# wreuven/h264-scroll-encoder

Measured on AMD Instinct MI355X. Metric: composed frames/sec (1280x720, 360x360 dyn) at 1/2/4/8 GPU; bit-exact vs CPU, higher is better.
Workload: dtype u8; 1 GPU; BASELINE config 3: 256 concurrent 1280x720 streams + 360x360 synthetic dynamic rect (4x4 int transform + quant + CAVLC), composer_write_scroll_frame semantics; resolution=1280x720, streams_per_gpu=256, parallelism=static stream shard x1, no RCCL

## Files before the change

h264-scroll-encoder_amd/csrc/dyn_engine.h:

```cpp
#ifndef SCROLL_DYN_ENGINE_H
#define SCROLL_DYN_ENGINE_H

#include <hip/hip_runtime.h>
#include "engine.h"

typedef struct {
    uint32_t *rows;
    uint16_t *meta;
    uint2 *body_lo, *body_hi;
    uint4 *body_w;
    uint4 *heads;
    unsigned long long *tcx;
    uint32_t *rowstage;
    uint32_t *gbits;
    uint32_t *spill;
    uint32_t *ctr;
    uint32_t ctr_frames;
    uint32_t epoch;
} DynScratch;
#define DYN_HEAD_VECS 16
#define DYN_CTR_LIST 4

typedef struct {
    hipStream_t side;
    hipEvent_t e0, e1;
} DynFork;
int dyn_launch_code(hipStream_t hs, int nframes, int S, DevStream *st, const NalDesc *nal,
                    int ld_nal, const PlanPending *pend, DynFrame *dfr, int ld_fr,
                    const DynGeom *g, const uint8_t *src, const uint8_t *refs, const DynScratch *x,
                    uint32_t epoch, int mbw, uint64_t *stamps, const DynFork *fk, hipEvent_t ev0 = nullptr,
                    hipEvent_t ev1 = nullptr);
int dyn_launch_static(hipStream_t hs, int nframes, int S, DevStream *st, const NalDesc *nal, int ld_nal,
                      const PlanPending *pend, DynFrame *dfr, int ld_fr, const DynGeom *g, const DynScratch *x);
int dyn_launch_pack(hipStream_t hs, int nframes, int S, DevStream *st, const NalDesc *nal,
                    int ld_nal, const PlanPending *pend, DynFrame *dfr, int ld_fr,
                    const DynGeom *g, const DynScratch *x, uint8_t *eps, uint64_t *stamps, const DynFork *fk);
int dyn_launch_emit(hipStream_t hs, int nframes, int S, const DevStream *st, const NalDesc *nal,
                    int ld_nal, const DynFrame *dfr, int ld_fr, const DynGeom *g,
                    const uint8_t *stage, const DynScratch *x, uint8_t *arena, uint64_t ld_arena,
                    uint64_t *stamps);
int dyn_launch_synth(hipStream_t hs, int nframes, int S, uint8_t *src, const DynGeom *g,
                     int stream_base, int t0);

void dyn_rowstage_geom(DynGeom *g, int mbw, int mbh);
size_t dyn_slot_bound(int mbw, int mbh, int rw, int rh);
uint32_t dyn_ep_cap(int rw, int rh, int debug);

#endif
```

h264-scroll-encoder_amd/csrc/dyn_kernels.hip:

```cpp
#include <hip/hip_runtime.h>

#include <stdint.h>
#include <mutex>

#include "dyn_device.h"
#include "dyn_engine.h"
#include "nal_ctx.h"
#include "row_mfma.h"
#include "stage_util.h"

using namespace scroll;
using namespace scroll::dyn;
using namespace scroll::stage;

namespace {

__constant__ Tabs g_tabs = SCROLL_DYN_TABS;
constexpr Tabs k_tabs = SCROLL_DYN_TABS;
__constant__ PTabs g_ptabs = make_ptabs(k_tabs);
__device__ uint32_t g_tzrb[TZRB_N];
__constant__ LvTab g_lvt = make_lvt();

struct QpPair {
    QParams l, c;
// ... 594 lines not shown

__device__ inline uint4 body_msb(uint64_t hi, uint64_t lo, uint32_t n)
{
    const uint32_t k = 128u - n;
    uint64_t H, Lw;
    if (k >= 64u) {
        H = k >= 128u ? 0ull : lo << (k - 64u);
        Lw = 0ull;
    } else {
        H = k ? (hi << k) | (lo >> (64u - k)) : hi;
        Lw = lo << k;
    }
    return make_uint4((uint32_t)(H >> 32), (uint32_t)H, (uint32_t)(Lw >> 32), (uint32_t)Lw);
}

__global__ __launch_bounds__(256) void k_dyn_rows(const DevStream *__restrict__ st,
                                                  const NalDesc *__restrict__ nal, int ld_nal,
                                                  const PlanPending *__restrict__ pend,
                                                  DynFrame *__restrict__ dfr, int ld_fr, DynGeom g,
                                                  uint32_t *__restrict__ rows, uint32_t *__restrict__ ctr,
                                                  uint4 *__restrict__ heads)
{
    __shared__ int32_t wo[8], wl[8], wv[8];
    __shared__ int32_t gen;
    const int s = blockIdx.y, f = blockIdx.x, t = threadIdx.x;
    DynFrame *DF = dfr + (size_t)s * ld_fr + f;
    const int j = DF->nal;
    if (j < 0) return;
    if (t < 8) {
        wo[t] = pend[s].wo[t];
        wl[t] = pend[s].wl[t];
        wv[t] = pend[s].wv[t];
    }
    if (t == 0) gen = 0;
    __syncthreads();
    const DevStream *S = st + s;
    const NalDesc d = nal[(size_t)s * ld_nal + j];
    const NalCtx c = nal_ctx(S, d, wo, wl, wv);
    if (t < 12) {
        const HeadCtx H = head_ctx(c);
        CapSink hc{0, 0, 0};
        H.put_class(hc, t);
        uint4 *hv = heads + ((size_t)s * ld_fr + f) * DYN_HEAD_VECS;
        hv[t] = body_msb(hc.hi, hc.lo, min(hc.n, 128u));
        reinterpret_cast<uint32_t *>(hv + 12)[t] = hc.n | (hc.over() ? 0x80000000u : 0u);
    }
    const Regions rg = regions(c);
    const int w = c.w, h = c.h, a_end = (h - c.off) / 16;
    const uint32_t ysz = (uint32_t)w * (uint32_t)h, pic = ysz + ysz / 2;
    const WpTab T{wo, wv, h};
    uint32_t *rw = rows + ((size_t)s * ld_fr + f) * (size_t)(32 * g.h);
    bool my_gen = false;
    for (int i = t; i < 32 * g.h; i += 256) {
        uint32_t e;
        if (i < 16 * g.h) {
            const int Y = 16 * g.y0 + i, row = Y >> 4;
            const bool cA = row < a_end;
            int yo;
            const int b = luma_row(T, cA ? rg.ra : rg.rb, Y + (cA ? rg.mva : rg.mvb), yo);
            e = (uint32_t)b * pic + (uint32_t)yo * (uint32_t)w;
        } else {
            const int i2 = i - 16 * g.h, bot = i2 >= 8 * g.h;
            const int Y = 8 * g.y0 + (bot ? i2 - 8 * g.h : i2), row = Y >> 3;
            const bool cA = row < a_end;
            const int q = 4 * (cA ? rg.mva : rg.mvb), o = q >> 3, fr = q & 7;
            int yo;
            const int b = chroma_row(T, cA ? rg.ra : rg.rb, Y + o + bot, yo);
            if (b < 0) {
// ... 10 lines not shown
    if (t == 0) {
        uint32_t e = 0u;
        if (gen) {
            const uint32_t k = atomicAdd(&ctr[1], 1u);
            if (k < g.gen_cap) {
                DF->rbsp_bytes = k;
                ctr[DYN_CTR_LIST + k] = (uint32_t)((size_t)s * ld_fr + f);
                e = DF_GENERAL;
            } else {
                e = DF_OVER;
            }
        }
        DF->err = e;
        DF->ep = 0u;
    }
}

constexpr int GW = 64;
#ifndef SCROLL_GBUF_WORDS
#define SCROLL_GBUF_WORDS 256
#endif
constexpr int GBUF_WORDS = SCROLL_GBUF_WORDS;

#ifndef SCROLL_STATIC_WORDS
#define SCROLL_STATIC_WORDS 1
#endif

struct StaticFixed {
    uint32_t ncand;
    uint32_t buf[GBUF_WORDS];
    uint64_t hhi[12], hlo[12];
    uint4 pat[12];
    uint32_t hlen[12];
    int32_t head_over;
    int32_t wo[8], wl[8], wv[8];
    uint32_t moff[DYN_STATIC_ROWS + 1];
};

__global__ __launch_bounds__(GW) void k_dyn_static(const DevStream *__restrict__ st,
                                                   const NalDesc *__restrict__ nal, int ld_nal,
                                                   const PlanPending *__restrict__ pend,
                                                   const DynFrame *__restrict__ dfr, int ld_fr, DynGeom g,
                                                   uint32_t *__restrict__ rowstage, uint32_t *__restrict__ gbits)
{
    __shared__ StaticFixed L;
    constexpr int SR = DYN_STATIC_ROWS;
    const Rect R{g.x0, g.y0, g.w, g.h};
    const int nA = max(1, (R.y0 + SR - 1) / SR);
    const int gi = (int)blockIdx.x >= nA ? (int)blockIdx.x + R.h : (int)blockIdx.x;
    const int ng = g.ngroups, f = blockIdx.y, s = blockIdx.z, t = threadIdx.x;
    const size_t nb = (size_t)s * ld_fr + f;
    const int j = dfr[nb].nal;
    if (j < 0) return;
    const bool first = gi == 0, last = gi == ng - 1;
    if (t < 8) {
        L.wo[t] = pend[s].wo[t];
        L.wl[t] = pend[s].wl[t];
        L.wv[t] = pend[s].wv[t];
    }
    if (t == 0) {
        L.head_over = 0;
        L.ncand = 0;
    }
    const DevStream *S = st + s;
    const NalDesc d = nal[(size_t)s * ld_nal + j];
    wave_sync();
    NalCtx c = nal_ctx(S, d, L.wo, L.wl, L.wv);
    c.qpd = S->dyn_qp - QP_DEFAULT;
    const HeadCtx H = head_ctx(c);
    const int mbw = H.mbw, mbh = c.h / 16;
    int ra, rb;
    if (gi < nA) {
        ra = gi * SR;
        rb = min(ra + SR, R.y0);
    } else {
        ra = R.y0 + R.h + (gi - nA - R.h) * SR;
        rb = min(ra + SR, mbh);
    }
    uint32_t F = 0;
    if (first) {
        CountSink hc{0};
        emit_slice_header(hc, c);
        F = hc.n;
    }
    if (t < 12) {
        CapSink hc{0, 0, 0};
        H.put_class(hc, t);
        L.hhi[t] = hc.hi;
        L.hlo[t] = hc.lo;
        L.hlen[t] = hc.n;
        if (hc.over()) L.head_over = 1;
        if (hc.n < 128u) {
            const uint64_t hi = (hc.hi << 1) | (hc.lo >> 63), lo = (hc.lo << 1) | 1u;
            L.pat[t] = body_msb(hi, lo, hc.n + 1u);
        } else {
            L.head_over = 1;
        }
    }
    wave_sync();
    const bool head_over = L.head_over;
    auto head_bits = [&](int r, int col) -> uint32_t {
        if (!head_over) return L.hlen[H.sel(r, col)];
        CountSink cn{0};
        H.put_slow(cn, r, col);
        return cn.n;
    };
    uint32_t len = 0;
    const int r = ra + t;
    if (r < rb) {
        if (!head_over) {
            len = row_static_bits(H, L.hlen, r, R);
        } else {
            for (int col = 0; col < mbw; ++col) len += head_bits(r, col) + 1u;
        }
    }
    const uint32_t incl = wave_incl_sum(len, t);
    if (r < rb) L.moff[r - ra] = F + incl - len;
    const uint32_t rows_end = F + __shfl(incl, GW - 1, GW);
    if (t == 0) L.moff[rb - ra] = rows_end;
    const uint32_t bits = rows_end + (last ? 1u : 0u);
    if (t == 0) gbits[nb * (size_t)ng + gi] = bits;
    wave_sync();

    uint32_t *out = rowstage + nb * g.rs_frame_words + rs_group_words(g, nA, gi);
    const uint32_t nw = min((bits + 31u) >> 5, g.rs_static_words - EPC_STATIC);
    const int ne = rb - ra;
    auto cnt_le = [&](uint32_t x) -> int {
        int lo = 0, hi = ne + 1;
        while (lo < hi) {
            const int mid = (lo + hi) >> 1;
            if (L.moff[mid] <= x) lo = mid + 1;
            else hi = mid;
        }
        return lo;
    };
    const uint32_t m_mbw = magic32((uint32_t)mbw);
    for (uint32_t p0 = 0; p0 < nw; p0 += GBUF_WORDS) {
        const uint32_t n = min((uint32_t)GBUF_WORDS, nw - p0);
        for (uint32_t i = (uint32_t)t; i < n; i += GW) L.buf[i] = 0u;
        wave_sync();
        const LdsOrWin win{L.buf, p0, n};
        if (!(SCROLL_STATIC_WORDS && !head_over) && first && t == 0 && p0 * 32u < F) {
            WSink hs{win, 0, 0, 0};
            hs.start(0);
            emit_slice_header(hs, c);
            hs.finish();
        }
        if (SCROLL_STATIC_WORDS && !head_over) {
            const uint32_t rbeg = L.moff[0], rend = L.moff[ne];
            for (uint32_t i = (uint32_t)t; i < n; i += GW) {
                const uint32_t W0 = 32u * (p0 + i), W1 = W0 + 32u;
                uint32_t acc = 0, b = max(W0, rbeg), R0 = 0, R1 = 0, L0 = 0, Lm = 1;
                int b3 = 0;
                float inv = 1.0f;
                while (b < W1 && b < rend) {
                    if (b >= R1 || b < R0) {
                        const int e = cnt_le(b) - 1;
                        R0 = L.moff[e];
                        R1 = L.moff[e + 1];
                        b3 = H.sel(ra + e, 0);
                        L0 = L.hlen[b3] + 1u;
                        Lm = L.hlen[b3 + 1] + 1u;
                        inv = 1.0f / (float)Lm;
                    }
                    const uint32_t o = b - R0;
                    uint32_t cl = (uint32_t)b3, off = o;
                    if (o >= L0) {
                        const uint32_t o2 = o - L0;
                        uint32_t q = (uint32_t)((float)o2 * inv);
                        if (q * Lm > o2) --q;
                        else if ((q + 1u) * Lm <= o2) ++q;
                        if (q < (uint32_t)(mbw - 2)) {
                            cl = (uint32_t)b3 + 1u;
                            off = o2 - q * Lm;
                        } else {
                            cl = (uint32_t)b3 + 2u;
                            off = o2 - (uint32_t)(mbw - 2) * Lm;
                        }
                    }
                    const uint32_t k = min(L.hlen[cl] + 1u - off, W1 - b);
                    const uint4 P = L.pat[cl];
                    const uint32_t wi = off >> 5, sh = off & 31u;
                    const uint32_t w0 = wi == 0 ? P.x : (wi == 1 ? P.y : (wi == 2 ? P.z : P.w));
                    const uint32_t w1 = wi == 0 ? P.y : (wi == 1 ? P.z : (wi == 2 ? P.w : 0u));
                    uint32_t v = sh ? __builtin_amdgcn_alignbit(w0, w1, 32u - sh) : w0;
                    v &= k >= 32u ? 0xffffffffu : ~(0xffffffffu >> k);
                    acc |= v >> (b - W0);
                    b += k;
                }
                L.buf[i] = acc;
            }
            wave_sync();
            if (first && t == 0 && p0 * 32u < F) {
                WSink hs{win, 0, 0, 0};
                hs.start(0);
                emit_slice_header(hs, c);
                hs.finish();
            }
            if (last && t == 0) {
                WSink sk{win, 0, 0, 0};
                sk.start(bits - 1u);
                sk.put(1, 1);
                sk.finish();
            }
            wave_sync();
            flush_window(L.buf, n, p0, p0 + n >= nw, out, &L.ncand,
                         rowstage + nb * g.rs_frame_words + rs_runs_words(g, nA, gi), EPC_STATIC - 1, t, GW);
            wave_sync();
            continue;
        }
        const int ea = max(cnt_le(32u * p0) - 1, 0), eb = min(cnt_le(32u * (p0 + n) - 1u), ne);
        const int nm = eb * mbw;
        for (int m = ea * mbw + t; m < nm; m += GW) {
            const int rr = (int)div_m((uint32_t)m, m_mbw), col = m - rr * mbw, rw = ra + rr;
            uint32_t off = L.moff[rr];
            WSink sk{win, 0, 0, 0};
            if (!head_over) {
                const int b3 = H.sel(rw, 0);
                off += col == 0 ? 0u : L.hlen[b3] + 1u + (uint32_t)(col - 1) * (L.hlen[b3 + 1] + 1u);
                if (off >= 32u * (p0 + n)) continue;
                const int cls = b3 + (col == 0 ? 0 : (col == mbw - 1 ? 2 : 1));
                if (off + L.hlen[cls] + 1u <= 32u * p0) continue;
                sk.start(off);
                sk.put_cap(CapSink{L.hhi[cls], L.hlo[cls], L.hlen[cls]});
            } else {
                for (int c2 = 0; c2 < col; ++c2) off += head_bits(rw, c2) + 1u;
                sk.start(off);
                H.put_slow(sk, rw, col);
            }
            sk.put(1, 1);
            sk.finish();
        }
        if (last && t == 0) {
            WSink sk{win, 0, 0, 0};
            sk.start(bits - 1u);
            sk.put(1, 1);
            sk.finish();
        }
        wave_sync();
        flush_window(L.buf, n, p0, p0 + n >= nw, out, &L.ncand,
                     rowstage + nb * g.rs_frame_words + rs_runs_words(g, nA, gi), EPC_STATIC - 1, t, GW);
        wave_sync();
    }
    if (t == 0) rowstage[nb * g.rs_frame_words + rs_runs_words(g, nA, gi)] = L.ncand;
}


__device__ inline CapSink cap_of_msb(uint64_t a, uint64_t b, uint32_t n)
{
    if (n == 0u) return CapSink{0, 0, 0};
    const uint32_t sh = 128u - n;
    if (sh >= 64u) return CapSink{0, a >> (sh - 64u), n};
    if (sh == 0u) return CapSink{a, b, n};
    return CapSink{a >> sh, (b >> sh) | (a << (64u - sh)), n};
}

__device__ inline void put_piece(uint32_t *buf, uint32_t p0, uint32_t n, uint32_t pos, uint32_t tv, uint32_t tl,
                                 uint4 b, uint32_t bl)
{
    const uint32_t tw = tv & low_mask((int)tl);
    const uint32_t c0 = __builtin_amdgcn_alignbit(tw, b.x, tl), c1 = __builtin_amdgcn_alignbit(b.x, b.y, tl);
// ... 2359 lines not shown
    } else {
        const uint32_t r = (i - ly) % (64u * (uint32_t)g.w * (uint32_t)g.h);
        const int cw = 8 * g.w;
        const int y = (int)(r / (uint32_t)cw), x = (int)(r - (uint32_t)(y * cw));
        const int X = 8 * g.x0 + x, Y = 8 * g.y0 + y;
        v = 128 + ((X + Y + (int)tt) & 15) - 8 + (int)(hv >> 30);
    }
    src[(size_t)s * g.src_ld + (size_t)f * g.src_fr + i] = (uint8_t)clampi(v, 0, 255);
}

}

int dyn_launch_code(hipStream_t hs, int nframes, int S, DevStream *st, const NalDesc *nal,
                    int ld_nal, const PlanPending *pend, DynFrame *dfr, int ld_fr,
                    const DynGeom *g, const uint8_t *src, const uint8_t *refs, const DynScratch *x,
                    uint32_t epoch, int mbw, uint64_t *stamps, const DynFork *fk, hipEvent_t ev0, hipEvent_t ev1)
{
    if (nframes <= 0 || S <= 0) return 0;
    {
        static std::mutex mu;
        static uint64_t ready = 0;
        int dev = 0;
        if (hipGetDevice(&dev) != hipSuccess || dev >= 64) return -1;
        std::lock_guard<std::mutex> lk(mu);
        if (!(ready >> dev & 1u)) {
            hipLaunchKernelGGL(k_tzrb_init, dim3((TZRB_N + 255) / 256), dim3(256), 0, hs);
            if (hipGetLastError() != hipSuccess || hipStreamSynchronize(hs) != hipSuccess) return -1;
            ready |= 1ull << dev;
        }
    }
    hipLaunchKernelGGL(k_dyn_rows, dim3(nframes, S), dim3(256), 0, hs, st, nal, ld_nal, pend, dfr, ld_fr,
                       *g, x->rows, x->ctr, x->heads);
    if (hipGetLastError() != hipSuccess) return -1;
    hipStream_t hg = hs;
    if (fk) {
        if (hipEventRecord(fk->e0, hs) != hipSuccess || hipStreamWaitEvent(fk->side, fk->e0, 0) != hipSuccess)
            return -1;
        hg = fk->side;
    }
    const int nchunk = (24 * g->w * g->h + CODE_T - 1) / CODE_T;
    hipLaunchKernelGGL(k_dyn_code_general, dim3(nchunk, CODE_GEN_Y), dim3(CODE_T), 0, hg, st, dfr, ld_fr,
                       pend, nal, ld_nal, *g, x->rows, src, refs, x->meta, x->body_lo, x->body_hi, x->body_w,
                       x->ctr);
    if (hipGetLastError() != hipSuccess) return -1;
    if (row_lds_bytes(g->w) > 65536) {
        const int rl = (int)row_lds_bytes(g->w);
        if (hipFuncSetAttribute(reinterpret_cast<const void *>(&k_dyn_row<false>),
                                hipFuncAttributeMaxDynamicSharedMemorySize, rl) != hipSuccess ||
            hipFuncSetAttribute(reinterpret_cast<const void *>(&k_dyn_row<true>),
                                hipFuncAttributeMaxDynamicSharedMemorySize, rl) != hipSuccess)
            return -1;
    }
    if (ev0 && hipEventRecord(ev0, hs) != hipSuccess) return -1;
    hipLaunchKernelGGL(k_dyn_row<false>, dim3(g->h, nframes, S), dim3(row_threads(g->w)),
                       row_lds_bytes(g->w), hs, st, nal, ld_nal, pend, dfr, ld_fr, *g, x->rows, src, refs,
                       x->meta, x->body_lo, x->body_hi, x->body_w, x->tcx, epoch, x->rowstage, x->gbits, x->spill,
                       x->ctr, x->heads, stamps);
    if (hipGetLastError() != hipSuccess) return -1;
    if (ev1 && hipEventRecord(ev1, hs) != hipSuccess) return -1;
    hipLaunchKernelGGL(k_dyn_row<true>, dim3(g->h, std::min<uint32_t>(g->gen_cap, (uint32_t)(nframes * S)), 1),
                       dim3(row_threads(g->w)),
                       row_lds_bytes(g->w), hg, st, nal, ld_nal, pend, dfr, ld_fr, *g, x->rows, src, refs,
                       x->meta, x->body_lo, x->body_hi, x->body_w, x->tcx, epoch, x->rowstage, x->gbits, x->spill,
                       x->ctr, x->heads, stamps);
    if (hipGetLastError() != hipSuccess) return -1;
    if (fk) {
        if (dyn_launch_static(hg, nframes, S, st, nal, ld_nal, pend, dfr, ld_fr, g, x) ||
            hipEventRecord(fk->e1, hg) != hipSuccess)
            return -1;
    }
    return 0;
}

int dyn_launch_static(hipStream_t hs, int nframes, int S, DevStream *st, const NalDesc *nal, int ld_nal,
                      const PlanPending *pend, DynFrame *dfr, int ld_fr, const DynGeom *g, const DynScratch *x)
{
    if (nframes <= 0 || S <= 0) return 0;
    hipLaunchKernelGGL(k_dyn_static, dim3(g->ngroups - g->h, nframes, S), dim3(GW), 0, hs, st, nal, ld_nal,
                       pend, dfr, ld_fr, *g, x->rowstage, x->gbits);
    return hipGetLastError() == hipSuccess ? 0 : -1;
}

int dyn_launch_pack(hipStream_t hs, int nframes, int S, DevStream *st, const NalDesc *nal,
                    int ld_nal, const PlanPending *pend, DynFrame *dfr, int ld_fr,
                    const DynGeom *g, const DynScratch *x, uint8_t *eps, uint64_t *stamps, const DynFork *fk)
{
    if (nframes <= 0 || S <= 0) return 0;
    if (fk) {
        if (hipStreamWaitEvent(hs, fk->e1, 0) != hipSuccess) return -1;
    } else if (dyn_launch_static(hs, nframes, S, st, nal, ld_nal, pend, dfr, ld_fr, g, x)) {
        return -1;
    }
    if (g->ep_cap >= (uint32_t)EPF_BIG_LIST)
        hipLaunchKernelGGL((k_dyn_epfix<EPF_T, EPF_BIG_LIST>), dim3(nframes, S), dim3(EPF_T), gtab_bytes(g->ngroups, true),
                           hs, st, dfr, ld_fr, nframes, *g, x->rowstage, x->gbits, eps, stamps);
    else
        hipLaunchKernelGGL((k_dyn_epfix<EPF_T, EPF_LIST>), dim3(nframes, S), dim3(EPF_T), gtab_bytes(g->ngroups, true),
                           hs, st, dfr, ld_fr, nframes, *g, x->rowstage, x->gbits, eps, stamps);
    return hipGetLastError() == hipSuccess ? 0 : -1;
}

int dyn_launch_emit(hipStream_t hs, int nframes, int S, const DevStream *st, const NalDesc *nal,
                    int ld_nal, const DynFrame *dfr, int ld_fr, const DynGeom *g,
                    const uint8_t *stage, const DynScratch *x, uint8_t *arena, uint64_t ld_arena,
                    uint64_t *stamps)
{
    if (nframes <= 0 || S <= 0) return 0;
// ... 70 lines not shown
```

h264-scroll-encoder_amd/csrc/scroll_kernels.hip:

```cpp
#include <hip/hip_runtime.h>

#include <stdarg.h>
#include <stdint.h>
#include <stdio.h>
#include <stdlib.h>
#include <string.h>

#include <algorithm>
#include <mutex>
#include <vector>

#include "dyn_engine.h"
#include "recon_engine.h"
#include "hrecon_engine.h"
#include "hint_engine.h"
#include "splice_engine.h"
#include "hdyn_engine.h"
#include "ingest_engine.h"
#include "ipcm_engine.h"
#include "engine.h"
#include "scroll_device.h"

#include "dyn_device.h"

// ... 809 lines not shown
    int hint_max_mb = 0;
    std::vector<std::vector<ScrollHintRect>> h_hint;
    std::vector<int16_t> h_hint_mode;
    HintFrame *d_hf = nullptr;
    ScrollHintRect *d_pool = nullptr;
    size_t pool_cap = 0;
    struct SpliceHost {
        int x0 = 0, y0 = 0, w = 0, h = 0;
        std::vector<uint8_t> nal;
        const uint8_t *dnal = nullptr;
        size_t n = 0;
    };
    std::vector<SpliceHost> h_sp;
    std::vector<int32_t> h_dyn_pos;
    int fallback = 0;
    DynFork fork{};
    std::vector<int32_t> h_dyn_qp;
    int dyn_pos_custom = 0;
    int dyn_qp = 26;
    int hd_dirty = 0;
    uint32_t hd_mb_words = 0;
    size_t dyn_cap = 0;
    int sp_n = 0;
    int sp_dirty = 0;
    int sp_parse = 0;
    SpliceFrame *d_spf = nullptr;
    uint8_t *d_sp_nal = nullptr;
    uint32_t *d_sp_rbsp = nullptr;
    SpliceMbRec *d_sp_rec = nullptr;
    int32_t *d_sp_list = nullptr;
    SpliceUnit *d_sp_units = nullptr;
// ... 124 lines not shown
    }
    memset(b->h_st, 0, S * sizeof(DevStream));
    b->last = b->own;
    *out = b;
    return SCROLL_OK;
}

void scroll_batch_destroy(ScrollBatch *b)
{
    if (!b) return;
    (void)hipSetDevice(b->device);
    if (b->own) (void)hipStreamSynchronize(b->own);
    for (int i = 0; i < NEV; ++i)
        if (b->ev[i]) (void)hipEventDestroy(b->ev[i]);
    for (hipEvent_t e : b->ring) (void)hipEventDestroy(e);
    if (b->fork.side) {
        (void)hipStreamSynchronize(b->fork.side);
        (void)hipStreamDestroy(b->fork.side);
        (void)hipEventDestroy(b->fork.e0);
        (void)hipEventDestroy(b->fork.e1);
    }
    if (b->own) (void)hipStreamDestroy(b->own);
    (void)hipFree(b->d_st);
    (void)hipHostFree(b->h_st);
    (void)hipFree(b->d_off);
    (void)hipFree(b->d_nal);
    (void)hipFree(b->d_arena);
    (void)hipFree(b->d_out_tab);
    (void)hipFree(b->d_upd);
    if (b->out_ev) (void)hipEventDestroy(b->out_ev);
    (void)hipFree(b->d_pend);
    (void)hipFree(b->d_dfr);
    (void)hipFree(b->d_src);
    (void)hipFree(b->d_refs);
    (void)hipFree(b->d_stage);
    (void)hipFree(b->d_rec);
// ... 278 lines not shown
                b->rc_timed = timed ? 1 : 0;
                b->rc_last_hint = 1;
                std::fill(b->rc_fail.begin(), b->rc_fail.end(), 0);
            }
            if ((b->sp_n > 0 || combined) &&
                splice_launch_stage(hs, nframes, S, b->d_st, b->d_nal, b->ld_nal, b->d_pend,
                                    b->d_dfr, ld_fr, b->d_hf, b->d_pool, b->d_spf, b->d_sp_rec,
                                    b->d_sp_rbsp, b->d_stage, b->geo.slot_bytes)) {
                set_err("k_splice_stage launch: %s", hipGetErrorString(hipGetLastError()));
                return SCROLL_ERR_HIP;
            }
            if ((rc = mark(6))) return rc;
        } else {
            b->dx.epoch = b->dx.epoch % 0xffffffu + 1u;
            const DynGeom &G = b->geo;
            const DynFork *fk = nullptr;
            static const bool fork_on = [] {
                const char *e = getenv("SCROLL_DYN_FORK");
                return e && e[0] == '1';
            }();
            if (fork_on) {
                if (!b->fork.side) {
                    HIPCHK(hipStreamCreateWithFlags(&b->fork.side, hipStreamNonBlocking));
                    HIPCHK(hipEventCreateWithFlags(&b->fork.e0, hipEventDisableTiming));
                    HIPCHK(hipEventCreateWithFlags(&b->fork.e1, hipEventDisableTiming));
                }
                fk = &b->fork;
            }
            if (dyn_launch_code(hs, nframes, S, b->d_st, b->d_nal, b->ld_nal, b->d_pend, b->d_dfr, ld_fr, &G,
                                b->d_src, b->d_refs, &b->dx, b->dx.epoch, b->dyn_pw / 16, stamps, fk,
                                lite_row ? rev[1] : nullptr, lite_row ? rev[6] : nullptr)) {
                set_err("k_dyn_code launch: %s", hipGetErrorString(hipGetLastError()));
                return SCROLL_ERR_HIP;
            }
            if ((rc = mark(6))) return rc;
            if (b->recon_on) {
                const bool timed = b->timing != 0;
                if (timed && !b->rc_ev[0]) {
                    HIPCHK(hipEventCreate(&b->rc_ev[0]));
                    HIPCHK(hipEventCreate(&b->rc_ev[1]));
                }
                if (recon_launch(hs, nframes, S, b->d_st, b->d_nal, b->ld_nal, b->d_pend, b->d_dfr, ld_fr, &G,
                                 b->dx.rows, b->d_src, b->d_refs, b->d_rec, b->d_sse, b->dx.ctr,
                                 timed ? b->rc_ev[0] : nullptr, timed ? b->rc_ev[1] : nullptr)) {
                    set_err("k_dyn_recon launch: %s", hipGetErrorString(hipGetLastError()));
                    return SCROLL_ERR_HIP;
                }
                b->rc_timed = timed ? 1 : 0;
                b->rc_last_hint = 0;
            }
            if (dyn_launch_pack(hs, nframes, S, b->d_st, b->d_nal, b->ld_nal, b->d_pend, b->d_dfr, ld_fr, &G,
                                &b->dx, b->d_stage, stamps ? b->d_dbg : nullptr, fk)) {
                set_err("k_dyn_static / k_dyn_epfix launch: %s", hipGetErrorString(hipGetLastError()));
                return SCROLL_ERR_HIP;
            }
        }
        if ((rc = mark(2))) return rc;
        hipLaunchKernelGGL(k_plan, dim3(S), dim3(PLAN_THREADS), 0, hs, b->d_st, b->d_off,
                           b->max_frames, b->d_nal, b->ld_nal, nframes, plan_mode,
                           b->debug | plan_flags | PLAN_SIZE | PLAN_DYN, b->d_pend, b->d_dfr,
                           ld_fr, (b->dyn_on && !b->hint_on) ? (const uint32_t *)b->dx.ctr : nullptr,
                           b->geo.rs_spill_cap, b->geo.gen_cap);
        HIPCHK(hipGetLastError());
        if ((rc = mark(3))) return rc;
    }
    int per_wg = EMIT_WAVES * TILE;
    int gx = (nal_max + per_wg - 1) / per_wg;
    if (gx > 0 && (b->debug & SCROLL_DEBUG_EMIT_STAMPS)) {
// ... 2161 lines not shown
```

Before: 2.875 million frames/s.

## Fuse static-group bitstream packing into k_dyn_rows and drop the side-stream fork

The separate k_dyn_static kernel, one 64-thread block per static row group, frame and stream, is folded into k_dyn_rows. The per-frame head classes are now computed once per block into shared StaticHeads, and each wave then processes static groups with its own dynamically sized LDS window. A precomputed repeated-pattern table (rep) lets the middle macroblocks of a row be copied in 32-bit chunks instead of pattern by pattern. The optional SCROLL_DYN_FORK side-stream path is removed. This cuts one launch and the repeated head-context setup per group, but the static work now runs serially before the general coder instead of possibly overlapping with it, and k_dyn_rows uses a variable block size chosen by rows_threads.

```diff
diff --git a/h264-scroll-encoder_amd/csrc/dyn_engine.h b/h264-scroll-encoder_amd/csrc/dyn_engine.h
--- a/h264-scroll-encoder_amd/csrc/dyn_engine.h
+++ b/h264-scroll-encoder_amd/csrc/dyn_engine.h
@@ -21,20 +21,13 @@
 #define DYN_HEAD_VECS 16
 #define DYN_CTR_LIST 4
 
-typedef struct {
-    hipStream_t side;
-    hipEvent_t e0, e1;
-} DynFork;
 int dyn_launch_code(hipStream_t hs, int nframes, int S, DevStream *st, const NalDesc *nal,
                     int ld_nal, const PlanPending *pend, DynFrame *dfr, int ld_fr,
                     const DynGeom *g, const uint8_t *src, const uint8_t *refs, const DynScratch *x,
-                    uint32_t epoch, int mbw, uint64_t *stamps, const DynFork *fk, hipEvent_t ev0 = nullptr,
+                    uint32_t epoch, int mbw, uint64_t *stamps, hipEvent_t ev0 = nullptr,
                     hipEvent_t ev1 = nullptr);
-int dyn_launch_static(hipStream_t hs, int nframes, int S, DevStream *st, const NalDesc *nal, int ld_nal,
-                      const PlanPending *pend, DynFrame *dfr, int ld_fr, const DynGeom *g, const DynScratch *x);
-int dyn_launch_pack(hipStream_t hs, int nframes, int S, DevStream *st, const NalDesc *nal,
-                    int ld_nal, const PlanPending *pend, DynFrame *dfr, int ld_fr,
-                    const DynGeom *g, const DynScratch *x, uint8_t *eps, uint64_t *stamps, const DynFork *fk);
+int dyn_launch_pack(hipStream_t hs, int nframes, int S, DevStream *st, DynFrame *dfr, int ld_fr,
+                    const DynGeom *g, const DynScratch *x, uint8_t *eps, uint64_t *stamps);
 int dyn_launch_emit(hipStream_t hs, int nframes, int S, const DevStream *st, const NalDesc *nal,
                     int ld_nal, const DynFrame *dfr, int ld_fr, const DynGeom *g,
                     const uint8_t *stage, const DynScratch *x, uint8_t *arena, uint64_t ld_arena,
diff --git a/h264-scroll-encoder_amd/csrc/dyn_kernels.hip b/h264-scroll-encoder_amd/csrc/dyn_kernels.hip
--- a/h264-scroll-encoder_amd/csrc/dyn_kernels.hip
+++ b/h264-scroll-encoder_amd/csrc/dyn_kernels.hip
@@ -632,15 +632,267 @@
     return make_uint4((uint32_t)(H >> 32), (uint32_t)H, (uint32_t)(Lw >> 32), (uint32_t)Lw);
 }
 
-__global__ __launch_bounds__(256) void k_dyn_rows(const DevStream *__restrict__ st,
+constexpr int GW = 64;
+#ifndef SCROLL_GBUF_WORDS
+#define SCROLL_GBUF_WORDS 256
+#endif
+constexpr int GBUF_WORDS = SCROLL_GBUF_WORDS;
+
+#ifndef SCROLL_STATIC_WORDS
+#define SCROLL_STATIC_WORDS 1
+#endif
+
+struct StaticHeads {
+    uint64_t hhi[12], hlo[12];
+    uint4 pat[12];
+    uint32_t hlen[12];
+    uint32_t rep[4][5];
+    int32_t head_over;
+};
+struct StaticWave {
+    uint32_t ncand;
+    uint32_t buf[GBUF_WORDS];
+    uint32_t moff[DYN_STATIC_ROWS + 1];
+};
+
+__device__ inline void static_rep_put(uint32_t *rp, uint4 P, uint32_t L)
+{
+    rp[0] = P.x;
+    rp[1] = P.y;
+    rp[2] = P.z;
+    rp[3] = P.w;
+    rp[4] = 0u;
+    for (uint32_t n = L; n < 160u; n <<= 1) {
+        const int ws = (int)(n >> 5);
+        const uint32_t bs = n & 31u;
+        uint32_t sft[5];
+#pragma unroll
+        for (int j = 0; j < 5; ++j) {
+            const int a = j - ws;
+            const uint32_t lo = a >= 0 ? rp[a] : 0u, hi = a >= 1 ? rp[a - 1] : 0u;
+            sft[j] = bs ? __builtin_amdgcn_alignbit(hi, lo, bs) : lo;
+        }
+#pragma unroll
+        for (int j = 0; j < 5; ++j) rp[j] |= sft[j];
+    }
+}
+
+__device__ inline void static_heads_put(StaticHeads &HD, int k, const CapSink &hc)
+{
+    HD.hhi[k] = hc.hi;
+    HD.hlo[k] = hc.lo;
+    HD.hlen[k] = hc.n;
+    if (hc.over()) HD.head_over = 1;
+    if (hc.n < 128u) {
+        const uint64_t hi = (hc.hi << 1) | (hc.lo >> 63), lo = (hc.lo << 1) | 1u;
+        HD.pat[k] = body_msb(hi, lo, hc.n + 1u);
+        if (k % 3 == 1) static_rep_put(HD.rep[k / 3], HD.pat[k], hc.n + 1u);
+    } else {
+        HD.head_over = 1;
+    }
+}
+
+__device__ inline void static_group(const StaticHeads &HD, StaticWave &L, const NalCtx &c, const HeadCtx &H,
+                                    const DynGeom &g, size_t nb, int gi, uint32_t *__restrict__ rowstage,
+                                    uint32_t *__restrict__ gbits, int t)
+{
+    constexpr int SR = DYN_STATIC_ROWS;
+    const Rect R{g.x0, g.y0, g.w, g.h};
+    const int nA = max(1, (R.y0 + SR - 1) / SR);
+    const int ng = g.ngroups;
+    const bool first = gi == 0, last = gi == ng - 1;
+    if (t == 0) L.ncand = 0;
+    const int mbw = H.mbw, mbh = c.h / 16;
+    int ra, rb;
+    if (gi < nA) {
+        ra = gi * SR;
+        rb = min(ra + SR, R.y0);
+    } else {
+        ra = R.y0 + R.h + (gi - nA - R.h) * SR;
+        rb = min(ra + SR, mbh);
+    }
+    uint32_t F = 0;
+    if (first) {
+        CountSink hc{0};
+        emit_slice_header(hc, c);
+        F = hc.n;
+    }
+    const bool head_over = HD.head_over;
+    auto head_bits = [&](int r, int col) -> uint32_t {
+        if (!head_over) return HD.hlen[H.sel(r, col)];
+        CountSink cn{0};
+        H.put_slow(cn, r, col);
+        return cn.n;
+    };
+    uint32_t len = 0;
+    const int r = ra + t;
+    if (r < rb) {
+        if (!head_over) {
+            len = row_static_bits(H, HD.hlen, r, R);
+        } else {
+            for (int col = 0; col < mbw; ++col) len += head_bits(r, col) + 1u;
+        }
+    }
+    const uint32_t incl = wave_incl_sum(len, t);
+    if (r < rb) L.moff[r - ra] = F + incl - len;
+    const uint32_t rows_end = F + __shfl(incl, GW - 1, GW);
+    if (t == 0) L.moff[rb - ra] = rows_end;
+    const uint32_t bits = rows_end + (last ? 1u : 0u);
+    if (t == 0) gbits[nb * (size_t)ng + gi] = bits;
+    wave_sync();
+
+    uint32_t *out = rowstage + nb * g.rs_frame_words + rs_group_words(g, nA, gi);
+    const uint32_t nw = min((bits + 31u) >> 5, g.rs_static_words - EPC_STATIC);
+    const int ne = rb - ra;
+    auto cnt_le = [&](uint32_t x) -> int {
+        int lo = 0, hi = ne + 1;
+        while (lo < hi) {
+            const int mid = (lo + hi) >> 1;
+            if (L.moff[mid] <= x) lo = mid + 1;
+            else hi = mid;
+        }
+        return lo;
+    };
+    const uint32_t m_mbw = magic32((uint32_t)mbw);
+    for (uint32_t p0 = 0; p0 < nw; p0 += GBUF_WORDS) {
+        const uint32_t n = min((uint32_t)GBUF_WORDS, nw - p0);
+        for (uint32_t i = (uint32_t)t; i < n; i += GW) L.buf[i] = 0u;
+        wave_sync();
+        const LdsOrWin win{L.buf, p0, n};
+        if (!(SCROLL_STATIC_WORDS && !head_over) && first && t == 0 && p0 * 32u < F) {
+            WSink hs{win, 0, 0, 0};
+            hs.start(0);
+            emit_slice_header(hs, c);
+            hs.finish();
+        }
+        if (SCROLL_STATIC_WORDS && !head_over) {
+            const uint32_t rbeg = L.moff[0], rend = L.moff[ne];
+            for (uint32_t i = (uint32_t)t; i < n; i += GW) {
+                const uint32_t W0 = 32u * (p0 + i), W1 = W0 + 32u;
+                uint32_t acc = 0, b = max(W0, rbeg), R0 = 0, R1 = 0, L0 = 0, Lm = 1;
+                int b3 = 0;
+                float inv = 1.0f;
+                while (b < W1 && b < rend) {
+                    if (b >= R1 || b < R0) {
+                        const int e = cnt_le(b) - 1;
+                        R0 = L.moff[e];
+                        R1 = L.moff[e + 1];
+                        b3 = H.sel(ra + e, 0);
+                        L0 = HD.hlen[b3] + 1u;
+                        Lm = HD.hlen[b3 + 1] + 1u;
+                        inv = 1.0f / (float)Lm;
+                    }
+                    const uint32_t o = b - R0;
+                    uint32_t cl = (uint32_t)b3, off = o;
+                    if (o >= L0) {
+                        const uint32_t o2 = o - L0, mid = (uint32_t)max(mbw - 2, 0) * Lm;
+                        if (o2 < mid) {
+                            uint32_t q = (uint32_t)((float)o2 * inv);
+                            if (q * Lm > o2) --q;
+                            else if ((q + 1u) * Lm <= o2) ++q;
+                            const uint32_t ph = o2 - q * Lm, k = min(mid - o2, W1 - b);
+                            const uint32_t *rp = HD.rep[b3 / 3];
+                            const uint32_t wi = ph >> 5, sh = ph & 31u;
+                            const uint32_t w0 = rp[wi], w1 = rp[wi + 1u];
+                            uint32_t v = sh ? __builtin_amdgcn_alignbit(w0, w1, 32u - sh) : w0;
+                            v &= k >= 32u ? 0xffffffffu : ~(0xffffffffu >> k);
+                            acc |= v >> (b - W0);
+                            b += k;
+                            continue;
+                        }
+                        cl = (uint32_t)b3 + 2u;
+                        off = o2 - mid;
+                    }
+                    const uint32_t k = min(HD.hlen[cl] + 1u - off, W1 - b);
+                    const uint4 P = HD.pat[cl];
+                    const uint32_t wi = off >> 5, sh = off & 31u;
+                    const uint32_t w0 = wi == 0 ? P.x : (wi == 1 ? P.y : (wi == 2 ? P.z : P.w));
+                    const uint32_t w1 = wi == 0 ? P.y : (wi == 1 ? P.z : (wi == 2 ? P.w : 0u));
+                    uint32_t v = sh ? __builtin_amdgcn_alignbit(w0, w1, 32u - sh) : w0;
+                    v &= k >= 32u ? 0xffffffffu : ~(0xffffffffu >> k);
+                    acc |= v >> (b - W0);
+                    b += k;
+                }
+                L.buf[i] = acc;
+            }
+            wave_sync();
+            if (first && t == 0 && p0 * 32u < F) {
+                WSink hs{win, 0, 0, 0};
+                hs.start(0);
+                emit_slice_header(hs, c);
+                hs.finish();
+            }
+            if (last && t == 0) {
+                WSink sk{win, 0, 0, 0};
+                sk.start(bits - 1u);
+                sk.put(1, 1);
+                sk.finish();
+            }
+            wave_sync();
+            flush_window(L.buf, n, p0, p0 + n >= nw, out, &L.ncand,
+                         rowstage + nb * g.rs_frame_words + rs_runs_words(g, nA, gi), EPC_STATIC - 1, t, GW);
+            wave_sync();
+            continue;
+        }
+        const int ea = max(cnt_le(32u * p0) - 1, 0), eb = min(cnt_le(32u * (p0 + n) - 1u), ne);
+        const int nm = eb * mbw;
+        for (int m = ea * mbw + t; m < nm; m += GW) {
+            const int rr = (int)div_m((uint32_t)m, m_mbw), col = m - rr * mbw, rw = ra + rr;
+            uint32_t off = L.moff[rr];
+            WSink sk{win, 0, 0, 0};
+            if (!head_over) {
+                const int b3 = H.sel(rw, 0);
+                off += col == 0 ? 0u : HD.hlen[b3] + 1u + (uint32_t)(col - 1) * (HD.hlen[b3 + 1] + 1u);
+                if (off >= 32u * (p0 + n)) continue;
+                const int cls = b3 + (col == 0 ? 0 : (col == mbw - 1 ? 2 : 1));
+                if (off + HD.hlen[cls] + 1u <= 32u * p0) continue;
+                sk.start(off);
+                sk.put_cap(CapSink{HD.hhi[cls], HD.hlo[cls], HD.hlen[cls]});
+            } else {
+                for (int c2 = 0; c2 < col; ++c2) off += head_bits(rw, c2) + 1u;
+                sk.start(off);
+                H.put_slow(sk, rw, col);
+            }
+            sk.put(1, 1);
+            sk.finish();
+        }
+        if (last && t == 0) {
+            WSink sk{win, 0, 0, 0};
+            sk.start(bits - 1u);
+            sk.put(1, 1);
+            sk.finish();
+        }
+        wave_sync();
+        flush_window(L.buf, n, p0, p0 + n >= nw, out, &L.ncand,
+                     rowstage + nb * g.rs_frame_words + rs_runs_words(g, nA, gi), EPC_STATIC - 1, t, GW);
+        wave_sync();
+    }
+    if (t == 0) rowstage[nb * g.rs_frame_words + rs_runs_words(g, nA, gi)] = L.ncand;
+    wave_sync();
+}
+
+constexpr int ROWS_MAXW = 8, ROWS_SLOTS = 8192;
+inline int rows_threads(const DynGeom &g, int64_t nnal)
+{
+    const int nst = g.ngroups - g.h;
+    int64_t maxw = nnal > 0 ? ROWS_SLOTS / nnal : ROWS_MAXW;
+    maxw = maxw < 1 ? 1 : (maxw > ROWS_MAXW ? ROWS_MAXW : maxw);
+    const int turns = (nst + (int)maxw - 1) / (int)maxw;
+    return 64 * ((nst + turns - 1) / turns);
+}
+__global__ __launch_bounds__(64 * ROWS_MAXW) __attribute__((amdgpu_waves_per_eu(8))) void k_dyn_rows(const DevStream *__restrict__ st,
                                                   const NalDesc *__restrict__ nal, int ld_nal,
                                                   const PlanPending *__restrict__ pend,
                                                   DynFrame *__restrict__ dfr, int ld_fr, DynGeom g,
                                                   uint32_t *__restrict__ rows, uint32_t *__restrict__ ctr,
-                                                  uint4 *__restrict__ heads)
+                                                  uint4 *__restrict__ heads, uint32_t *__restrict__ rowstage,
+                                                  uint32_t *__restrict__ gbits)
 {
     __shared__ int32_t wo[8], wl[8], wv[8];
     __shared__ int32_t gen;
+    __shared__ StaticHeads HD;
+    extern __shared__ __attribute__((aligned(16))) uint8_t rows_dyn[];
+    StaticWave *SW = reinterpret_cast<StaticWave *>(rows_dyn);
     const int s = blockIdx.y, f = blockIdx.x, t = threadIdx.x;
     DynFrame *DF = dfr + (size_t)s * ld_fr + f;
     const int j = DF->nal;
@@ -650,7 +902,10 @@
         wl[t] = pend[s].wl[t];
         wv[t] = pend[s].wv[t];
     }
-    if (t == 0) gen = 0;
+    if (t == 0) {
+        gen = 0;
+        HD.head_over = 0;
+    }
     __syncthreads();
     const DevStream *S = st + s;
     const NalDesc d = nal[(size_t)s * ld_nal + j];
@@ -662,6 +917,7 @@
         uint4 *hv = heads + ((size_t)s * ld_fr + f) * DYN_HEAD_VECS;
         hv[t] = body_msb(hc.hi, hc.lo, min(hc.n, 128u));
         reinterpret_cast<uint32_t *>(hv + 12)[t] = hc.n | (hc.over() ? 0x80000000u : 0u);
+        static_heads_put(HD, t, hc);
     }
     const Regions rg = regions(c);
     const int w = c.w, h = c.h, a_end = (h - c.off) / 16;
@@ -669,7 +925,7 @@
     const WpTab T{wo, wv, h};
     uint32_t *rw = rows + ((size_t)s * ld_fr + f) * (size_t)(32 * g.h);
     bool my_gen = false;
-    for (int i = t; i < 32 * g.h; i += 256) {
+    for (int i = t; i < 32 * g.h; i += (int)blockDim.x) {
         uint32_t e;
         if (i < 16 * g.h) {
             const int Y = 16 * g.y0 + i, row = Y >> 4;
@@ -710,237 +966,18 @@
         DF->err = e;
         DF->ep = 0u;
     }
-}
-
-constexpr int GW = 64;
-#ifndef SCROLL_GBUF_WORDS
-#define SCROLL_GBUF_WORDS 256
-#endif
-constexpr int GBUF_WORDS = SCROLL_GBUF_WORDS;
-
-#ifndef SCROLL_STATIC_WORDS
-#define SCROLL_STATIC_WORDS 1
-#endif
-
-struct StaticFixed {
-    uint32_t ncand;
-    uint32_t buf[GBUF_WORDS];
-    uint64_t hhi[12], hlo[12];
-    uint4 pat[12];
-    uint32_t hlen[12];
-    int32_t head_over;
-    int32_t wo[8], wl[8], wv[8];
-    uint32_t moff[DYN_STATIC_ROWS + 1];
-};
-
-__global__ __launch_bounds__(GW) void k_dyn_static(const DevStream *__restrict__ st,
-                                                   const NalDesc *__restrict__ nal, int ld_nal,
-                                                   const PlanPending *__restrict__ pend,
-                                                   const DynFrame *__restrict__ dfr, int ld_fr, DynGeom g,
-                                                   uint32_t *__restrict__ rowstage, uint32_t *__restrict__ gbits)
-{
-    __shared__ StaticFixed L;
-    constexpr int SR = DYN_STATIC_ROWS;
-    const Rect R{g.x0, g.y0, g.w, g.h};
-    const int nA = max(1, (R.y0 + SR - 1) / SR);
-    const int gi = (int)blockIdx.x >= nA ? (int)blockIdx.x + R.h : (int)blockIdx.x;
-    const int ng = g.ngroups, f = blockIdx.y, s = blockIdx.z, t = threadIdx.x;
-    const size_t nb = (size_t)s * ld_fr + f;
-    const int j = dfr[nb].nal;
-    if (j < 0) return;
-    const bool first = gi == 0, last = gi == ng - 1;
-    if (t < 8) {
-        L.wo[t] = pend[s].wo[t];
-        L.wl[t] = pend[s].wl[t];
-        L.wv[t] = pend[s].wv[t];
-    }
-    if (t == 0) {
-        L.head_over = 0;
-        L.ncand = 0;
-    }
-    const DevStream *S = st + s;
-    const NalDesc d = nal[(size_t)s * ld_nal + j];
-    wave_sync();
-    NalCtx c = nal_ctx(S, d, L.wo, L.wl, L.wv);
-    c.qpd = S->dyn_qp - QP_DEFAULT;
-    const HeadCtx H = head_ctx(c);
-    const int mbw = H.mbw, mbh = c.h / 16;
-    int ra, rb;
-    if (gi < nA) {
-        ra = gi * SR;
-        rb = min(ra + SR, R.y0);
-    } else {
-        ra = R.y0 + R.h + (gi - nA - R.h) * SR;
-        rb = min(ra + SR, mbh);
-    }
-    uint32_t F = 0;
-    if (first) {
-        CountSink hc{0};
-        emit_slice_header(hc, c);
-        F = hc.n;
-    }
-    if (t < 12) {
-        CapSink hc{0, 0, 0};
-        H.put_class(hc, t);
-        L.hhi[t] = hc.hi;
-        L.hlo[t] = hc.lo;
-        L.hlen[t] = hc.n;
-        if (hc.over()) L.head_over = 1;
-        if (hc.n < 128u) {
-            const uint64_t hi = (hc.hi << 1) | (hc.lo >> 63), lo = (hc.lo << 1) | 1u;
-            L.pat[t] = body_msb(hi, lo, hc.n + 1u);
-        } else {
-            L.head_over = 1;
-        }
-    }
-    wave_sync();
-    const bool head_over = L.head_over;
-    auto head_bits = [&](int r, int col) -> uint32_t {
-        if (!head_over) return L.hlen[H.sel(r, col)];
-        CountSink cn{0};
-        H.put_slow(cn, r, col);
-        return cn.n;
-    };
-    uint32_t len = 0;
-    const int r = ra + t;
-    if (r < rb) {
-        if (!head_over) {
-            len = row_static_bits(H, L.hlen, r, R);
-        } else {
-            for (int col = 0; col < mbw; ++col) len += head_bits(r, col) + 1u;
-        }
-    }
-    const uint32_t incl = wave_incl_sum(len, t);
-    if (r < rb) L.moff[r - ra] = F + incl - len;
-    const uint32_t rows_end = F + __shfl(incl, GW - 1, GW);
-    if (t == 0) L.moff[rb - ra] = rows_end;
-    const uint32_t bits = rows_end + (last ? 1u : 0u);
-    if (t == 0) gbits[nb * (size_t)ng + gi] = bits;
-    wave_sync();
-
-    uint32_t *out = rowstage + nb * g.rs_frame_words + rs_group_words(g, nA, gi);
-    const uint32_t nw = min((bits + 31u) >> 5, g.rs_static_words - EPC_STATIC);
-    const int ne = rb - ra;
-    auto cnt_le = [&](uint32_t x) -> int {
-        int lo = 0, hi = ne + 1;
-        while (lo < hi) {
-            const int mid = (lo + hi) >> 1;
-            if (L.moff[mid] <= x) lo = mid + 1;
-            else hi = mid;
-        }
-        return lo;
-    };
-    const uint32_t m_mbw = magic32((uint32_t)mbw);
-    for (uint32_t p0 = 0; p0 < nw; p0 += GBUF_WORDS) {
-        const uint32_t n = min((uint32_t)GBUF_WORDS, nw - p0);
-        for (uint32_t i = (uint32_t)t; i < n; i += GW) L.buf[i] = 0u;
-        wave_sync();
-        const LdsOrWin win{L.buf, p0, n};
-        if (!(SCROLL_STATIC_WORDS && !head_over) && first && t == 0 && p0 * 32u < F) {
-            WSink hs{win, 0, 0, 0};
-            hs.start(0);
-            emit_slice_header(hs, c);
-            hs.finish();
-        }
-        if (SCROLL_STATIC_WORDS && !head_over) {
-            const uint32_t rbeg = L.moff[0], rend = L.moff[ne];
-            for (uint32_t i = (uint32_t)t; i < n; i += GW) {
-                const uint32_t W0 = 32u * (p0 + i), W1 = W0 + 32u;
-                uint32_t acc = 0, b = max(W0, rbeg), R0 = 0, R1 = 0, L0 = 0, Lm = 1;
-                int b3 = 0;
-                float inv = 1.0f;
-                while (b < W1 && b < rend) {
-                    if (b >= R1 || b < R0) {
-                        const int e = cnt_le(b) - 1;
-                        R0 = L.moff[e];
-                        R1 = L.moff[e + 1];
-                        b3 = H.sel(ra + e, 0);
-                        L0 = L.hlen[b3] + 1u;
-                        Lm = L.hlen[b3 + 1] + 1u;
-                        inv = 1.0f / (float)Lm;
-                    }
-                    const uint32_t o = b - R0;
-                    uint32_t cl = (uint32_t)b3, off = o;
-                    if (o >= L0) {
-                        const uint32_t o2 = o - L0;
-                        uint32_t q = (uint32_t)((float)o2 * inv);
-                        if (q * Lm > o2) --q;
-                        else if ((q + 1u) * Lm <= o2) ++q;
-                        if (q < (uint32_t)(mbw - 2)) {
-                            cl = (uint32_t)b3 + 1u;
-                            off = o2 - q * Lm;
-                        } else {
-                            cl = (uint32_t)b3 + 2u;
-                            off = o2 - (uint32_t)(mbw - 2) * Lm;
-                        }
-                    }
-                    const uint32_t k = min(L.hlen[cl] + 1u - off, W1 - b);
-                    const uint4 P = L.pat[cl];
-                    const uint32_t wi = off >> 5, sh = off & 31u;
-                    const uint32_t w0 = wi == 0 ? P.x : (wi == 1 ? P.y : (wi == 2 ? P.z : P.w));
-                    const uint32_t w1 = wi == 0 ? P.y : (wi == 1 ? P.z : (wi == 2 ? P.w : 0u));
-                    uint32_t v = sh ? __builtin_amdgcn_alignbit(w0, w1, 32u - sh) : w0;
-                    v &= k >= 32u ? 0xffffffffu : ~(0xffffffffu >> k);
-                    acc |= v >> (b - W0);
-                    b += k;
-                }
-                L.buf[i] = acc;
-            }
-            wave_sync();
-            if (first && t == 0 && p0 * 32u < F) {
-                WSink hs{win, 0, 0, 0};
-                hs.start(0);
-                emit_slice_header(hs, c);
-                hs.finish();
-            }
-            if (last && t == 0) {
-                WSink sk{win, 0, 0, 0};
-                sk.start(bits - 1u);
-                sk.put(1, 1);
-                sk.finish();
-            }
-            wave_sync();
-            flush_window(L.buf, n, p0, p0 + n >= nw, out, &L.ncand,
-                         rowstage + nb * g.rs_frame_words + rs_runs_words(g, nA, gi), EPC_STATIC - 1, t, GW);
-            wave_sync();
-            continue;
-        }
-        const int ea = max(cnt_le(32u * p0) - 1, 0), eb = min(cnt_le(32u * (p0 + n) - 1u), ne);
-        const int nm = eb * mbw;
-        for (int m = ea * mbw + t; m < nm; m += GW) {
-            const int rr = (int)div_m((uint32_t)m, m_mbw), col = m - rr * mbw, rw = ra + rr;
-            uint32_t off = L.moff[rr];
-            WSink sk{win, 0, 0, 0};
-            if (!head_over) {
-                const int b3 = H.sel(rw, 0);
-                off += col == 0 ? 0u : L.hlen[b3] + 1u + (uint32_t)(col - 1) * (L.hlen[b3 + 1] + 1u);
-                if (off >= 32u * (p0 + n)) continue;
-                const int cls = b3 + (col == 0 ? 0 : (col == mbw - 1 ? 2 : 1));
-                if (off + L.hlen[cls] + 1u <= 32u * p0) continue;
-                sk.start(off);
-                sk.put_cap(CapSink{L.hhi[cls], L.hlo[cls], L.hlen[cls]});
-            } else {
-                for (int c2 = 0; c2 < col; ++c2) off += head_bits(rw, c2) + 1u;
-                sk.start(off);
-                H.put_slow(sk, rw, col);
-            }
-            sk.put(1, 1);
-            sk.finish();
-        }
-        if (last && t == 0) {
-            WSink sk{win, 0, 0, 0};
-            sk.start(bits - 1u);
-            sk.put(1, 1);
-            sk.finish();
-        }
-        wave_sync();
-        flush_window(L.buf, n, p0, p0 + n >= nw, out, &L.ncand,
-                     rowstage + nb * g.rs_frame_words + rs_runs_words(g, nA, gi), EPC_STATIC - 1, t, GW);
-        wave_sync();
-    }
-    if (t == 0) rowstage[nb * g.rs_frame_words + rs_runs_words(g, nA, gi)] = L.ncand;
-}
-
+    {
+        constexpr int SR = DYN_STATIC_ROWS;
+        const int nA = max(1, (g.y0 + SR - 1) / SR), nst = g.ngroups - g.h;
+        const int nwv = (int)blockDim.x >> 6, wave = t >> 6;
+        NalCtx cs = c;
+        cs.qpd = S->dyn_qp - QP_DEFAULT;
+        const HeadCtx H = head_ctx(cs);
+        for (int k = nwv - 1 - wave; k < nst; k += nwv)
+            static_group(HD, SW[wave], cs, H, g, (size_t)s * ld_fr + f, k >= nA ? k + g.h : k, rowstage, gbits,
+                         t & 63);
+    }
+}
 
 __device__ inline CapSink cap_of_msb(uint64_t a, uint64_t b, uint32_t n)
 {
@@ -3330,7 +3367,7 @@
 int dyn_launch_code(hipStream_t hs, int nframes, int S, DevStream *st, const NalDesc *nal,
                     int ld_nal, const PlanPending *pend, DynFrame *dfr, int ld_fr,
                     const DynGeom *g, const uint8_t *src, const uint8_t *refs, const DynScratch *x,
-                    uint32_t epoch, int mbw, uint64_t *stamps, const DynFork *fk, hipEvent_t ev0, hipEvent_t ev1)
+                    uint32_t epoch, int mbw, uint64_t *stamps, hipEvent_t ev0, hipEvent_t ev1)
 {
     if (nframes <= 0 || S <= 0) return 0;
     {
@@ -3345,17 +3382,12 @@
             ready |= 1ull << dev;
         }
     }
-    hipLaunchKernelGGL(k_dyn_rows, dim3(nframes, S), dim3(256), 0, hs, st, nal, ld_nal, pend, dfr, ld_fr,
-                       *g, x->rows, x->ctr, x->heads);
+    const int rt = rows_threads(*g, (int64_t)nframes * S);
+    hipLaunchKernelGGL(k_dyn_rows, dim3(nframes, S), dim3(rt), (size_t)(rt / 64) * sizeof(StaticWave), hs, st, nal,
+                       ld_nal, pend, dfr, ld_fr, *g, x->rows, x->ctr, x->heads, x->rowstage, x->gbits);
     if (hipGetLastError() != hipSuccess) return -1;
-    hipStream_t hg = hs;
-    if (fk) {
-        if (hipEventRecord(fk->e0, hs) != hipSuccess || hipStreamWaitEvent(fk->side, fk->e0, 0) != hipSuccess)
-            return -1;
-        hg = fk->side;
-    }
     const int nchunk = (24 * g->w * g->h + CODE_T - 1) / CODE_T;
-    hipLaunchKernelGGL(k_dyn_code_general, dim3(nchunk, CODE_GEN_Y), dim3(CODE_T), 0, hg, st, dfr, ld_fr,
+    hipLaunchKernelGGL(k_dyn_code_general, dim3(nchunk, CODE_GEN_Y), dim3(CODE_T), 0, hs, st, dfr, ld_fr,
                        pend, nal, ld_nal, *g, x->rows, src, refs, x->meta, x->body_lo, x->body_hi, x->body_w,
                        x->ctr);
     if (hipGetLastError() != hipSuccess) return -1;
@@ -3376,37 +3408,17 @@
     if (ev1 && hipEventRecord(ev1, hs) != hipSuccess) return -1;
     hipLaunchKernelGGL(k_dyn_row<true>, dim3(g->h, std::min<uint32_t>(g->gen_cap, (uint32_t)(nframes * S)), 1),
                        dim3(row_threads(g->w)),
-                       row_lds_bytes(g->w), hg, st, nal, ld_nal, pend, dfr, ld_fr, *g, x->rows, src, refs,
+                       row_lds_bytes(g->w), hs, st, nal, ld_nal, pend, dfr, ld_fr, *g, x->rows, src, refs,
                        x->meta, x->body_lo, x->body_hi, x->body_w, x->tcx, epoch, x->rowstage, x->gbits, x->spill,
                        x->ctr, x->heads, stamps);
     if (hipGetLastError() != hipSuccess) return -1;
-    if (fk) {
-        if (dyn_launch_static(hg, nframes, S, st, nal, ld_nal, pend, dfr, ld_fr, g, x) ||
-            hipEventRecord(fk->e1, hg) != hipSuccess)
-            return -1;
-    }
     return 0;
 }
 
-int dyn_launch_static(hipStream_t hs, int nframes, int S, DevStream *st, const NalDesc *nal, int ld_nal,
-                      const PlanPending *pend, DynFrame *dfr, int ld_fr, const DynGeom *g, const DynScratch *x)
+int dyn_launch_pack(hipStream_t hs, int nframes, int S, DevStream *st, DynFrame *dfr, int ld_fr,
+                    const DynGeom *g, const DynScratch *x, uint8_t *eps, uint64_t *stamps)
 {
     if (nframes <= 0 || S <= 0) return 0;
-    hipLaunchKernelGGL(k_dyn_static, dim3(g->ngroups - g->h, nframes, S), dim3(GW), 0, hs, st, nal, ld_nal,
-                       pend, dfr, ld_fr, *g, x->rowstage, x->gbits);
-    return hipGetLastError() == hipSuccess ? 0 : -1;
-}
-
-int dyn_launch_pack(hipStream_t hs, int nframes, int S, DevStream *st, const NalDesc *nal,
-                    int ld_nal, const PlanPending *pend, DynFrame *dfr, int ld_fr,
-                    const DynGeom *g, const DynScratch *x, uint8_t *eps, uint64_t *stamps, const DynFork *fk)
-{
-    if (nframes <= 0 || S <= 0) return 0;
-    if (fk) {
-        if (hipStreamWaitEvent(hs, fk->e1, 0) != hipSuccess) return -1;
-    } else if (dyn_launch_static(hs, nframes, S, st, nal, ld_nal, pend, dfr, ld_fr, g, x)) {
-        return -1;
-    }
     if (g->ep_cap >= (uint32_t)EPF_BIG_LIST)
         hipLaunchKernelGGL((k_dyn_epfix<EPF_T, EPF_BIG_LIST>), dim3(nframes, S), dim3(EPF_T), gtab_bytes(g->ngroups, true),
                            hs, st, dfr, ld_fr, nframes, *g, x->rowstage, x->gbits, eps, stamps);
diff --git a/h264-scroll-encoder_amd/csrc/scroll_kernels.hip b/h264-scroll-encoder_amd/csrc/scroll_kernels.hip
--- a/h264-scroll-encoder_amd/csrc/scroll_kernels.hip
+++ b/h264-scroll-encoder_amd/csrc/scroll_kernels.hip
@@ -847,7 +847,6 @@
     std::vector<SpliceHost> h_sp;
     std::vector<int32_t> h_dyn_pos;
     int fallback = 0;
-    DynFork fork{};
     std::vector<int32_t> h_dyn_qp;
     int dyn_pos_custom = 0;
     int dyn_qp = 26;
@@ -1002,12 +1001,6 @@
     for (int i = 0; i < NEV; ++i)
         if (b->ev[i]) (void)hipEventDestroy(b->ev[i]);
     for (hipEvent_t e : b->ring) (void)hipEventDestroy(e);
-    if (b->fork.side) {
-        (void)hipStreamSynchronize(b->fork.side);
-        (void)hipStreamDestroy(b->fork.side);
-        (void)hipEventDestroy(b->fork.e0);
-        (void)hipEventDestroy(b->fork.e1);
-    }
     if (b->own) (void)hipStreamDestroy(b->own);
     (void)hipFree(b->d_st);
     (void)hipHostFree(b->h_st);
@@ -1316,21 +1309,8 @@
         } else {
             b->dx.epoch = b->dx.epoch % 0xffffffu + 1u;
             const DynGeom &G = b->geo;
-            const DynFork *fk = nullptr;
-            static const bool fork_on = [] {
-                const char *e = getenv("SCROLL_DYN_FORK");
-                return e && e[0] == '1';
-            }();
-            if (fork_on) {
-                if (!b->fork.side) {
-                    HIPCHK(hipStreamCreateWithFlags(&b->fork.side, hipStreamNonBlocking));
-                    HIPCHK(hipEventCreateWithFlags(&b->fork.e0, hipEventDisableTiming));
-                    HIPCHK(hipEventCreateWithFlags(&b->fork.e1, hipEventDisableTiming));
-                }
-                fk = &b->fork;
-            }
             if (dyn_launch_code(hs, nframes, S, b->d_st, b->d_nal, b->ld_nal, b->d_pend, b->d_dfr, ld_fr, &G,
-                                b->d_src, b->d_refs, &b->dx, b->dx.epoch, b->dyn_pw / 16, stamps, fk,
+                                b->d_src, b->d_refs, &b->dx, b->dx.epoch, b->dyn_pw / 16, stamps,
                                 lite_row ? rev[1] : nullptr, lite_row ? rev[6] : nullptr)) {
                 set_err("k_dyn_code launch: %s", hipGetErrorString(hipGetLastError()));
                 return SCROLL_ERR_HIP;
@@ -1351,9 +1331,9 @@
                 b->rc_timed = timed ? 1 : 0;
                 b->rc_last_hint = 0;
             }
-            if (dyn_launch_pack(hs, nframes, S, b->d_st, b->d_nal, b->ld_nal, b->d_pend, b->d_dfr, ld_fr, &G,
-                                &b->dx, b->d_stage, stamps ? b->d_dbg : nullptr, fk)) {
-                set_err("k_dyn_static / k_dyn_epfix launch: %s", hipGetErrorString(hipGetLastError()));
+            if (dyn_launch_pack(hs, nframes, S, b->d_st, b->d_dfr, ld_fr, &G, &b->dx, b->d_stage,
+                                stamps ? b->d_dbg : nullptr)) {
+                set_err("k_dyn_epfix launch: %s", hipGetErrorString(hipGetLastError()));
                 return SCROLL_ERR_HIP;
             }
         }
```

New measurement: 2.895 million frames/s (median of 6 runs). Within noise of the previous version (+0.7%).
